# shaia/CFD

Measured on AMD Instinct MI355X. Metric: MLUPS + achieved HBM GB/s, 512^3 projection step, 1/2/4/8xMI355X, higher is better.
Workload: dtype f64

## Files before the change

### cfd_amd/csrc/hip/ccf.hpp

```cpp
#pragma once

#include "kernels.hpp"

namespace cfdhip {

#ifndef CFD_CCF_AHEAD
#define CFD_CCF_AHEAD 2
#endif
constexpr int CCF_AHEAD = CFD_CCF_AHEAD;
static_assert(CCF_AHEAD == 1 || CCF_AHEAD == 2, "k_ccf prefetch depth");
#ifndef CFD_CCF_CFIRST
#define CFD_CCF_CFIRST 0
#endif
constexpr bool CCF_CFIRST = CFD_CCF_CFIRST != 0;
#ifndef CFD_CCF_DIAG
#define CFD_CCF_DIAG 0
#endif
constexpr int CCF_DIAG = CFD_CCF_DIAG;
#ifndef CFD_CCF_NTST
#define CFD_CCF_NTST 1
#endif
constexpr bool CCF_NTST = CFD_CCF_NTST != 0;
#ifndef CFD_CCF_STAUX
#define CFD_CCF_STAUX (CFD_CCF_NTST ? 2 : 0)
#endif
constexpr int CCF_STAUX = CFD_CCF_STAUX;
#ifndef CFD_CCF_LDAUX
#define CFD_CCF_LDAUX 0
#endif
constexpr int CCF_LDAUX = CFD_CCF_LDAUX;
#ifndef CFD_CCF_NTFOLD
#define CFD_CCF_NTFOLD 0
#endif
constexpr bool CCF_NTFOLD = CFD_CCF_NTFOLD != 0;
constexpr int CCF_TC = 32;
constexpr int CCF_TR = 32;
constexpr int CCF_OX = 60;
constexpr int CCF_OY = 28;
constexpr int CCF_LP = CCF_TC + 2;
constexpr int CCF_LR = 2 * CCF_LP;
constexpr int CCF_LS = (CCF_TR + 2) * CCF_LR;
struct CcfLds {
    double pl[4][CCF_LS];
    double sh[32];
    int flag;
};

template <bool FIRST, bool FOLD, bool NOC = false>
static __global__ __launch_bounds__(1024, 4) void k_ccf(
    SGeo g, Lap Lp, const double* __restrict__ R0, double* __restrict__ R1,
    const double* __restrict__ Po, double* __restrict__ Pn, PPrev pv, double* __restrict__ x,
    CgState* st, double* partials, unsigned* counter, int it, int xmap, int dist, double* dsum,
    Mbox* mb, unsigned long long* clk) {
    static_assert(!(FIRST && FOLD), "k_ccf: no fold in the first iteration");
    __shared__ CcfLds L;
    if (CCF_DIAG == 0 && st->done) return;
    unsigned long long clk_t0 = 0, clk_r0 = 0;
    if (clk != nullptr && threadIdx.x < 64) {
        clk_t0 = __builtin_amdgcn_s_memtime();
        clk_r0 = __builtin_amdgcn_s_memrealtime();
        __builtin_amdgcn_s_waitcnt(0xC07F);
    }
    const double a = st->alpha[it % CG_XFOLD];
    const double ma = -a;
    const double beta = FIRST ? 0.0 : st->beta;
    double aq[CG_XFOLD - 1];
#pragma unroll
    for (int q = 0; q < CG_XFOLD - 1; ++q)
        aq[q] = FOLD ? st->alpha[(it + 1 + q) % CG_XFOLD] : 0.0;
    const int t = xmap ? xcd_tile(blockIdx.x, gridDim.x) : (int)blockIdx.x;
    const int tx = t % g.tiles_x;
    const int rest = t / g.tiles_x;
    const int ty = rest % g.tiles_y;
    const int tz = rest / g.tiles_y;
    const int lane = threadIdx.x & 63;
    const int w = __builtin_amdgcn_readfirstlane(threadIdx.x >> 6);
    const int c = lane & 31;
    const int r = w + 16 * (lane >> 5);
    const int i0 = tx * CCF_OX - 2 + 2 * c;
    const int j = ty * CCF_OY - 2 + r;
    int kb, ke;
    if (g.kmode == 1) {
        kb = (tz == 0) ? g.k0 : g.k1 - 1;
        ke = kb + 1;
    } else {
        const int kt0 = (g.kmode == 2) ? g.kt0 : g.k0;
        const int kt1 = (g.kmode == 2) ? g.kt1 : g.k1;
        if (tz < g.nz1) {
            kb = kt0 + tz * g.kc;
            ke = min(kb + g.kc, kt1);
        } else {
            kb = min(kt0 + g.nz1 * g.kc + (tz - g.nz1) * g.kc2, kt1);
            ke = min(kb + g.kc2, kt1);
        }
    }
    const bool jin = j >= 1 && j <= g.ny - 2;
    const bool in0 = jin && i0 >= 1 && i0 <= g.nx - 2;
    const bool in1 = jin && i0 + 1 >= 1 && i0 + 1 <= g.nx - 2;
    const bool own = c >= 1 && c <= CCF_TC - 2 && r >= 2 && r <= CCF_TR - 3;
    const bool wr = own && jin && i0 >= 0 && i0 < g.nx;
    const int ic = i0 < 0 ? 0 : (i0 < g.nx ? i0 : g.nx - 2 - ((g.nx - 2) & 1));
    const int col = max(min(j, g.ny - 1), 0) * (int)g.px + ic;
    auto plane = [&](int k) -> long long {
        return CCF_DIAG == 1 ? 0LL : (long long)min(max(k, 0), g.nz - 1) * g.ps;
    };
    double* const Lb = &L.pl[0][r * CCF_LR + c];
    constexpr int OWX = CCF_LR + 1, OWY = CCF_LR + 1 + CCF_LP;
    constexpr int LFo = CCF_LR + CCF_LP, RTo = CCF_LR + 2;
    constexpr int DNX = 1, DNY = 1 + CCF_LP, UPX = 2 * CCF_LR + 1, UPY = 2 * CCF_LR + 1 + CCF_LP;
    auto lrd = [&](int pl, int d) __attribute__((always_inline)) -> double {
        __builtin_amdgcn_sched_barrier(0x7ff);
        return Lb[pl * CCF_LS + d];
    };
    auto lput = [&](int pl, double2 v) __attribute__((always_inline)) {
        Lb[pl * CCF_LS + OWX] = v.x;
        Lb[pl * CCF_LS + OWY] = v.y;
    };
    for (int e = threadIdx.x; e < 4 * CCF_LS; e += 1024) {
        const int q = e % CCF_LS;
        const int row = q / CCF_LR, cc = q % CCF_LP;
        if (row == 0 || row == CCF_TR + 1 || cc == 0 || cc == CCF_LP - 1) L.pl[e / CCF_LS][q] = 0.0;
    }
    struct Nb {
        double lf, rt, dx, dy, ux, uy;
    };
    auto nbrs = [&](int pl) __attribute__((always_inline)) -> Nb {
        Nb n;
        n.lf = lrd(pl, LFo);
        n.rt = lrd(pl, RTo);
        n.dx = lrd(pl, DNX);
        n.dy = lrd(pl, DNY);
        n.ux = lrd(pl, UPX);
        n.uy = lrd(pl, UPY);
        return n;
    };
    auto stencil_n = [&](const Nb& n, double2 v, double2 zm, double2 zp, double2& out)
                         __attribute__((always_inline)) {
        out.x = -lap7(Lp, v.x, n.lf, v.y, n.dx, n.ux, zm.x, zp.x);
        out.y = -lap7(Lp, v.y, v.x, n.rt, n.dy, n.uy, zm.y, zp.y);
    };
    auto stencil = [&](int pl, double2 v, double2 zm, double2 zp, double2& out)
                       __attribute__((always_inline)) {
        if constexpr (CCF_DIAG == 2) {
            out.x = v.x + zm.x + zp.x;
            out.y = v.y + zm.y + zp.y;
        } else {
            stencil_n(nbrs(pl), v, zm, zp, out);
        }
    };
    const int q0 = kb - 4;
    const int nsteps = ke - kb + 4;
    double2 rr[4], po[4], pn[4], rn[4];
    double2 fx[2], f0[2], f1[2];
    const double2 zero = make_double2(0.0, 0.0);
#pragma unroll
    for (int s = 0; s < 4; ++s) pn[s] = rn[s] = po[s] = rr[s] = zero;
    fx[0] = fx[1] = f0[0] = f0[1] = f1[0] = f1[1] = zero;
    auto pro = [&](int k) __attribute__((always_inline)) {
        const int s = (k - q0) & 3;
        rr[s] = ld2ba<CCF_LDAUX>(R0 + plane(k), g.ps, col * 8);
        if (!FIRST) po[s] = ld2ba<CCF_LDAUX>(Po + plane(k), g.ps, col * 8);
        st2b<false>(Pn, g.ps, ST_NOSTORE, zero);
        st2b<false>(R1, g.ps, ST_NOSTORE, zero);
        if (FOLD) st2b<false>(x, g.ps, ST_NOSTORE, zero);
        __builtin_amdgcn_sched_barrier(0);
    };
    rr[2] = po[2] = zero;
    pro(q0 + 2);
    if (CCF_AHEAD == 2) pro(q0 + 3);
    double accg = 0.0, accd = 0.0;
    auto step = [&](auto Pc, int q) __attribute__((always_inline)) {
        constexpr int P = decltype(Pc)::value;
        constexpr int S0 = P & 3, S1 = (P + 1) & 3, S2 = (P + 2) & 3, S3 = (P + 3) & 3;
        constexpr int SM = (P + 3) & 3;
        constexpr int F1 = (P + 1) & 1, F2 = P & 1;
        constexpr int LPR = (P + 1) & 1, LPW = P & 1;
        constexpr int LRR = 2 + (P & 1), LRW = 2 + ((P + 1) & 1);
        __builtin_amdgcn_sched_barrier(0);
        {
            constexpr int SL = (CCF_AHEAD == 2) ? S0 : S3;
            const int ql = q + CCF_AHEAD + 2;
            const long long pbl = plane(ql);
            const int ol = (ql <= ke + 1) ? col * 8 : ST_NOSTORE;
            rr[SL] = ld2ba<CCF_LDAUX>(R0 + pbl, g.ps, ol);
            if (!FIRST) po[SL] = ld2ba<CCF_LDAUX>(Po + pbl, g.ps, ol);
        }
        if (FOLD) {
            const long long pb2 = plane(q + 2);
            const int o2 = (wr && q + 2 >= kb && q + 2 < ke) ? col * 8 : ST_NOSTORE;
            fx[F2] = ld2b<CCF_NTFOLD>(x + pb2, g.ps, o2);
            f0[F2] = ld2b<CCF_NTFOLD>(pv.q[0] + pb2, g.ps, o2);
            f1[F2] = ld2b<CCF_NTFOLD>(pv.q[1] + pb2, g.ps, o2);
        }
        __builtin_amdgcn_sched_barrier(0);
        __syncthreads();
        Nb nc{};
        if constexpr (!NOC && CCF_CFIRST) nc = nbrs(LRR);
        const double2 p2 = FIRST ? rr[S2] : fma2p(rr[S2], beta, po[S2]);
        pn[S2] = p2;
        double2 s;
        stencil(LPR, pn[S1], pn[S0], p2, s);
        const int qb = q + 1;
        const bool kbin = qb >= 1 && qb <= g.nz - 2;
        const double2 rv = rr[S1];
        const double2 r1 = make_double2((kbin && in0) ? rv.x + ma * s.x : 0.0,
                                        (kbin && in1) ? rv.y + ma * s.y : 0.0);
        rn[S1] = r1;
        if constexpr (!CCF_CFIRST) __builtin_amdgcn_sched_barrier(0);
        if constexpr (!NOC) {
            double2 wv;
            if constexpr (CCF_CFIRST) stencil_n(nc, rn[S0], rn[SM], r1, wv);
            else stencil(LRR, rn[S0], rn[SM], r1, wv);
            if (q >= kb && own) {
                const double2 rc = rn[S0];
                if (in0) {
                    accg += rc.x * rc.x;
                    accd += wv.x * rc.x;
                }
                if (in1) {
                    accg += rc.y * rc.y;
                    accd += wv.y * rc.y;
                }
            }
        }
        lput(LPW, p2);
        if constexpr (!NOC) lput(LRW, r1);
        {
            const bool qown = qb >= kb && qb < ke;
            const int bo = (qown && wr && CCF_DIAG != 1) ? col * 8 : ST_NOSTORE;
            const bool qhalo = NOC && ((qb == kb - 1 && kb == g.k0) || (qb == ke && ke == g.k1));
            const int bp = ((qown || qhalo) && wr && CCF_DIAG != 1) ? col * 8 : ST_NOSTORE;
            const long long pb = plane(qb);
            const double2 p1 = pn[S1];
            st2ba<CCF_STAUX>(Pn + pb, g.ps, bp, make_double2(in0 ? p1.x : 0.0, in1 ? p1.y : 0.0));
            st2ba<CCF_STAUX>(R1 + pb, g.ps, bo, r1);
            if (FOLD) {
                const double2 xo = fx[F1], qa = f0[F1], qq = f1[F1], qc = po[S1];
                double2 xw;
                xw.x = in0 ? (((xo.x + aq[0] * qa.x) + aq[1] * qq.x) + aq[2] * qc.x) + a * p1.x
                           : xo.x;
                xw.y = in1 ? (((xo.y + aq[0] * qa.y) + aq[1] * qq.y) + aq[2] * qc.y) + a * p1.y
                           : xo.y;
                st2ba<CCF_STAUX>(x + pb, g.ps, bo, xw);
            }
        }
        __builtin_amdgcn_sched_barrier(0);
    };
    int n = 0;
    for (; n + 3 < nsteps; n += 4) {
        step(IntC<0>{}, q0 + n);
        step(IntC<1>{}, q0 + n + 1);
        step(IntC<2>{}, q0 + n + 2);
        step(IntC<3>{}, q0 + n + 3);
    }
    if (n < nsteps) step(IntC<0>{}, q0 + n);
    if (n + 1 < nsteps) step(IntC<1>{}, q0 + n + 1);
    if (n + 2 < nsteps) step(IntC<2>{}, q0 + n + 2);
    if (clk != nullptr && threadIdx.x < 64) {
        const unsigned long long t1 = __builtin_amdgcn_s_memtime();
        const unsigned long long r1 = __builtin_amdgcn_s_memrealtime();
        __builtin_amdgcn_s_waitcnt(0xC07F);
        if (threadIdx.x == 0) {
            atomicAdd(&clk[0], t1 - clk_t0);
            atomicAdd(&clk[1], r1 - clk_r0);
            atomicAdd(&clk[2], 1ull);
        }
    }
    if constexpr (NOC) return;
    accg = wave_sum(accg);
    accd = wave_sum(accd);
    __syncthreads();
    if (lane == 0) {
        L.sh[w] = accg;
        L.sh[16 + w] = accd;
    }
    __syncthreads();
    double bg = 0.0, bd = 0.0;
    if (threadIdx.x == 0)
        for (int v = 0; v < 16; ++v) {
            bg += L.sh[v];
            bd += L.sh[16 + v];
        }
    double tg, td;
    double* shs = &L.pl[0][0];
    if (grid_sum2_last<1024>(bg, bd, partials, counter, shs, &L.flag, tg, td,
                             (unsigned)g.part_ofs, (unsigned)g.part_total) &&
        threadIdx.x == 0)
        cc_reduce_finish(st, tg, td, it, false, dist != 0, mb, dsum);
}

}
```

### cfd_amd/csrc/hip/ctx.hpp

```cpp
#pragma once

#include "kernels.hpp"
#include "slab_comm.hpp"

#include "cfd_hip/projection_hip.h"

#include <hip/hip_ext.h>
#include <hip/hip_runtime.h>

#include <algorithm>
#include <cmath>
#include <cstdio>
#include <cstdlib>
#include <cstring>
#include <initializer_list>
#include <vector>

using namespace cfdhip;

extern "C" void cfd_set_error(cfd_status_t status, const char* message) __attribute__((weak));

static inline void set_err(cfd_status_t s, const char* msg) {
    if (cfd_set_error) cfd_set_error(s, msg);
}
// ... 6 lines not shown
            snprintf(buf_, sizeof(buf_), "HIP error %s at %s:%d (%s)",             \
                     hipGetErrorString(e_), __FILE__, __LINE__, #call);            \
            set_err(CFD_ERROR, buf_);                                              \
            return CFD_ERROR;                                                      \
        }                                                                          \
    } while (0)

namespace {

struct TimedLaunch {
    hipEvent_t a, b;
    int kind;
    int iter;
};

}

struct hip_proj_ctx {
    int device = 0;
    hipStream_t stream = nullptr;
    size_t nx = 0, ny = 0, nz = 0;
    long long px = 0, ps = 0;
    Geo geo{};
    SGeo sgeo{};
    SGeo sg_edge{}, sg_int{};
    SGeo rgeo{};
    SGeo rg_in1{}, rg_edge{}, rg_in2{};
    int split_rb = 0;
    SGeo rg_main{}, rg_strip{};
    int rb_strip_tc = 0;
    int rb1_tc = 64;
    SGeo pgeo{};
    SGeo pgeo16{};
    int pc3 = 1;
    int split_b = 0;
    int sweep_ty = 8;
    int sweep_variant = 0;
    int sweep_variant_fold = 0;
    int grid_cap = 2048;
    hip_proj_config_t cfg{};
    SlabComm* comm = nullptr;
    int rank = 0, nranks = 1;
    size_t nzg = 0;
    size_t kofs = 0;
    double* dsum = nullptr;
    unsigned long long* clk = nullptr;
    hipStream_t hstream = nullptr;
    hipEvent_t ev_b = nullptr, ev_h = nullptr;
    unsigned long long* redg = nullptr;
    double *u = nullptr, *v = nullptr, *w = nullptr, *p = nullptr, *T = nullptr;
    double *us = nullptr, *vs = nullptr, *ws = nullptr, *pn = nullptr;
    double *r = nullptr, *pa = nullptr, *pb = nullptr;
    double *pc4 = nullptr, *pd4 = nullptr;
    double *rhs = nullptr, *xt = nullptr;
    int cg_scratch_dirty = 0;
    int poisson_bc = 0;
    double* bcfix = nullptr;
    int resident = 0;
    const double* res_ptr[5] = {nullptr, nullptr, nullptr, nullptr, nullptr};
    long long res_steps = 0;
    unsigned long long host_hash[5] = {0, 0, 0, 0, 0};
    unsigned long long host_hash1[5] = {0, 0, 0, 0, 0};
    int hash_ok = 0, hash_nf = 0;
    double* shell_dev = nullptr;
    double* shell_host = nullptr;
    size_t shell_cap = 0;
    double *cw = nullptr, *cs = nullptr;
    double* Tn = nullptr;
    double* rho = nullptr;
    double* rk_acc[4] = {nullptr, nullptr, nullptr, nullptr};
    double *dxa = nullptr, *dya = nullptr;
    double *src_u_row = nullptr, *src_v_col = nullptr;
    double* h_src = nullptr;
    hipEvent_t ev_src = nullptr;
    CgState* st = nullptr;
    RxState* rxst = nullptr;
    RxState* rxst2 = nullptr;
    void* rb2dec = nullptr;
    SGeo r2geo{};
    SGeo ccgeo{};
    SGeo cc_edge{}, cc_int{};
    SGeo cc_int_red{}, cc2_edge{};
    int ccf_tail = 0, ccf_kc2 = 0;
    std::vector<float> placement_ms;
    int placement_pick = -1;
    double* r2 = nullptr;
    double* partials = nullptr;
    unsigned* counter = nullptr;
    unsigned long long* red = nullptr;
    CgState* h_state = nullptr;
    unsigned long long* h_red = nullptr;
    hipEvent_t ev_poll[2] = {nullptr, nullptr};
    double rho0 = 1.0;
    double max_T = 0.0;
    int have_T = 0;
    int T_dirty = 0;
    poisson_solver_stats_t pstats{};
    size_t bytes = 0;
    std::vector<void*> allocs;
    size_t stagger_bytes = 0;
    struct {
        bool ccf_off = false;
        int cg_small = -1;
        int rb2_test = 0;
        int rb2_xmap = 0;
        bool rb2_log = false;
        int rb2 = 1;
        int ccf_xmap = 0;
        bool cgb_rev = true;
        bool rb1_pf = true;
        bool rb1_alt = true;
        bool rb1_fold = true;
        bool rk_pair = true;
        bool alloc_contig = false;
        bool ccf_edge_side = true;
    } env;
    int timing = 0;
    std::vector<hipEvent_t> ev_pool;
    size_t ev_used = 0;
    std::vector<TimedLaunch> pending;
    hipEvent_t ta = nullptr, tb = nullptr;
    double kt_ms[HIP_KT_COUNT] = {0};
    long long kt_n[HIP_KT_COUNT] = {0};
};

static cfd_status_t dalloc(hip_proj_ctx* c, double** ptr, size_t n) {
    const size_t off = (size_t)c->allocs.size() * c->stagger_bytes;
    void* base = nullptr;
    if (c->env.alloc_contig &&
        hipExtMallocWithFlags(&base, n * sizeof(double) + off, hipDeviceMallocContiguous) != hipSuccess) {
        (void)hipGetLastError();
        base = nullptr;
    }
    if (!base) HIP_TRY(hipMalloc(&base, n * sizeof(double) + off));
    c->allocs.push_back(base);
    *ptr = (double*)((char*)base + off);
    HIP_TRY(hipMemsetAsync(*ptr, 0, n * sizeof(double), c->stream));
    c->bytes += n * sizeof(double) + off;
    return CFD_SUCCESS;
}

static size_t field_elems(const hip_proj_ctx* c) { return (size_t)c->ps * c->nz; }

static double* field_ptr(hip_proj_ctx* c, int id) {
    switch (id) {
        case HIP_FIELD_U: return c->u;
        case HIP_FIELD_V: return c->v;
        case HIP_FIELD_W: return c->w;
        case HIP_FIELD_P: return c->p;
        case HIP_FIELD_T: return c->T;
        case HIP_FIELD_RHO: return c->rho;
        default: return nullptr;
    }
}

static hipEvent_t take_event(hip_proj_ctx* c) {
    if (c->ev_used == c->ev_pool.size()) {
        hipEvent_t e;
        if (hipEventCreate(&e) != hipSuccess) return nullptr;
        c->ev_pool.push_back(e);
    }
    return c->ev_pool[c->ev_used++];
}

static void flush_timing(hip_proj_ctx* c, int cg_limit = 0x7fffffff) {
    for (auto& t : c->pending) {
        if (t.iter >= cg_limit) continue;
        float ms = 0.f;
        if (hipEventElapsedTime(&ms, t.a, t.b) == hipSuccess) {
            c->kt_ms[t.kind] += ms;
            c->kt_n[t.kind] += 1;
        }
    }
    c->pending.clear();
    c->ev_used = 0;
}

template <typename F>
static void timed(hip_proj_ctx* c, int kind, F&& launch, int iter = -1) {
    if (!c->timing) {
        launch();
        return;
    }
    hipEvent_t a = take_event(c), b = take_event(c);
    if (!a || !b) {
        launch();
        return;
    }
    c->ta = a;
    c->tb = b;
    launch();
    c->ta = c->tb = nullptr;
    c->pending.push_back({a, b, kind, iter});
}

template <typename F>
static cfd_status_t timed_span(hip_proj_ctx* c, hipStream_t s, int kind, F&& fn, int iter = -1) {
    if (!c->timing) return fn();
// ... 143 lines not shown
```

### cfd_amd/csrc/hip/projection_hip.hip

```cpp
#include "ctx.hpp"

#include <array>
#include "rb2.hpp"
#include "ccf.hpp"

template <int TY, bool FIRST, bool DIST, int FL, bool FOLD>
static void launch_cgA_t(hip_proj_ctx* c, const Lap& L, const double* r, const double* po,
                         double* pn, int it, const PFold& fd) {
    hipExtLaunchKernelGGL((k_cgA<TY, FIRST, DIST, FL, FOLD>), dim3(sweep_grid(c)), dim3(64 * TY),
                          0, c->stream, c->ta, c->tb, 0, c->sgeo, L, r, po, pn, c->st, c->partials,
                          c->counter, it, c->dsum, mbox(c), fd);
}

struct BArgs {
    const double* p;
    double* r;
};

template <int TY, bool DIST, int FL>
static void launch_cgB_t(hip_proj_ctx* c, const SGeo& sg, const Lap& L, const BArgs& a, int it) {
    const unsigned nb = (unsigned)(sg.tiles_x * sg.tiles_y * sg.tiles_z);
    if (!DIST && c->env.cgb_rev && c->geo.sz && sg.kmode == 0) {
        hipExtLaunchKernelGGL((k_cgB<TY, DIST, FL, true>), dim3(nb), dim3(64 * TY), 0, c->stream,
                              c->ta, c->tb, 0, sg, L, a.p, a.r, c->st, c->partials, c->counter,
// ... 51 lines not shown
        case 4: return launch_cgB_f<TY, 4>(c, sg, L, a, it);
        case 7: return launch_cgB_f<TY, 7>(c, sg, L, a, it);
        case 15: return launch_cgB_f<TY, 15>(c, sg, L, a, it);
                 [[fallthrough]];
        case 23: if constexpr (TY == 16) return launch_cgB_f<TY, 23>(c, sg, L, a, it);
                 [[fallthrough]];
        case 31: if constexpr (TY == 16) return launch_cgB_f<TY, 31>(c, sg, L, a, it);
                 [[fallthrough]];
        default: return launch_cgB_f<TY, 0>(c, sg, L, a, it);
    }
}

static void launch_cgA(hip_proj_ctx* c, bool first, const Lap& L, const double* r,
                       const double* po, double* pn, int it, const PFold& fd) {
    if (c->sweep_ty == 4) return launch_cgA_f<4, 0>(c, first, L, r, po, pn, it, fd);
    if (c->sweep_ty == 16) return launch_cgA_v<16>(c, first, L, r, po, pn, it, fd);
    return launch_cgA_v<8>(c, first, L, r, po, pn, it, fd);
}

static void launch_cgB(hip_proj_ctx* c, const SGeo& sg, const Lap& L, const BArgs& a, int it) {
    if (c->sweep_ty == 4) return launch_cgB_f<4, 0>(c, sg, L, a, it);
    if (c->sweep_ty == 16) return launch_cgB_v<16>(c, sg, L, a, it);
    return launch_cgB_v<8>(c, sg, L, a, it);
}

template <bool FIRST, bool FOLD>
static void launch_cc1_t(hip_proj_ctx* c, double* pn, const double* po, const PPrev& pv, double* x,
                         int it) {
    const unsigned n = (unsigned)(c->px / 2) * (unsigned)(c->ny - 2) *
                       (unsigned)(c->sgeo.k1 - c->sgeo.k0);
    const unsigned nb = std::max(1u, std::min((n + 255) / 256, (unsigned)c->grid_cap * 4));
    hipExtLaunchKernelGGL((k_cc1<FIRST, FOLD>), dim3(nb), dim3(256), 0, c->stream, c->ta, c->tb, 0,
                          c->sgeo, c->r, c->cw, c->cs, po, pn, pv, x, c->st, it);
}

static void launch_cc1(hip_proj_ctx* c, double* pn, const double* po, const PPrev& pv, double* x,
                       int it) {
    const bool fold = (it % CG_XFOLD) == CG_XFOLD - 1;
    if (it == 0) launch_cc1_t<true, false>(c, pn, po, pv, x, it);
    else if (fold) launch_cc1_t<false, true>(c, pn, po, pv, x, it);
    else launch_cc1_t<false, false>(c, pn, po, pv, x, it);
}

template <int TY, bool DIST, bool INIT, bool WST>
static void launch_cc2_t(hip_proj_ctx* c, const SGeo& g, const Lap& L, int it, const double* r) {
    const unsigned nb = (unsigned)(g.tiles_x * g.tiles_y * g.tiles_z);
    hipExtLaunchKernelGGL((k_cc2<TY, DIST, INIT, WST>), dim3(nb), dim3(64 * TY), 0,
                          c->stream, c->ta, c->tb, 0, g, L, r, c->cw, c->st, c->partials,
                          c->counter, it, c->dsum, mbox(c));
}

template <int TY, bool WST>
static void launch_cc2_w(hip_proj_ctx* c, const SGeo& g, const Lap& L, int it, bool init,
                         const double* r) {
    if (dist(c)) init ? launch_cc2_t<TY, true, true, WST>(c, g, L, it, r)
                      : launch_cc2_t<TY, true, false, WST>(c, g, L, it, r);
    else init ? launch_cc2_t<TY, false, true, WST>(c, g, L, it, r)
              : launch_cc2_t<TY, false, false, WST>(c, g, L, it, r);
}

template <int TY>
static void launch_cc2_ty(hip_proj_ctx* c, const SGeo& g, const Lap& L, int it, bool init,
                          const double* r, bool wst) {
    wst ? launch_cc2_w<TY, true>(c, g, L, it, init, r)
        : launch_cc2_w<TY, false>(c, g, L, it, init, r);
}

static void launch_cc2(hip_proj_ctx* c, const Lap& L, int it, bool init, const double* r,
                       bool wst, const SGeo* gp = nullptr) {
    const SGeo& g = gp ? *gp : c->sgeo;
    if (c->sweep_ty == 16) return launch_cc2_ty<16>(c, g, L, it, init, r, wst);
    if (c->sweep_ty == 4) return launch_cc2_ty<4>(c, g, L, it, init, r, wst);
    return launch_cc2_ty<8>(c, g, L, it, init, r, wst);
}

static const double* ccf_r0(const hip_proj_ctx* c, int it) { return (it & 1) ? c->r2 : c->r; }
static double* ccf_r1(hip_proj_ctx* c, int it) { return (it & 1) ? c->r : c->r2; }

template <bool FIRST, bool FOLD, bool NOC>
static void launch_ccf_t(hip_proj_ctx* c, const SGeo& g, const Lap& L, double* pn,
                         const double* po, const PPrev& pv, double* x, int it, int xmap,
                         hipStream_t s) {
    unsigned long long* clk = (c->timing && c->clk && (it & 5) == 5) ? c->clk : nullptr;
    hipExtLaunchKernelGGL((k_ccf<FIRST, FOLD, NOC>), dim3(g.tiles_x * g.tiles_y * g.tiles_z),
                          dim3(1024), 0, s, c->ta, c->tb, 0, g, L, ccf_r0(c, it),
                          ccf_r1(c, it), po, pn, pv, x, c->st, c->partials, c->counter, it, xmap,
                          dist(c) ? 1 : 0, c->dsum, mbox(c), clk);
}

template <bool NOC>
static void launch_ccf_n(hip_proj_ctx* c, const SGeo& g, const Lap& L, double* pn,
                         const double* po, const PPrev& pv, double* x, int it, int xmap,
                         hipStream_t s) {
    const bool fold = (it % CG_XFOLD) == CG_XFOLD - 1;
    if (it == 0) launch_ccf_t<true, false, NOC>(c, g, L, pn, po, pv, x, it, xmap, s);
    else if (fold) launch_ccf_t<false, true, NOC>(c, g, L, pn, po, pv, x, it, xmap, s);
    else launch_ccf_t<false, false, NOC>(c, g, L, pn, po, pv, x, it, xmap, s);
}

static void launch_ccf(hip_proj_ctx* c, const SGeo& g, const Lap& L, double* pn,
                       const double* po, const PPrev& pv, double* x, int it, bool noc,
                       hipStream_t s = nullptr) {
    const int xmap = c->env.ccf_xmap;
    if (!s) s = c->stream;
    if (noc) launch_ccf_n<true>(c, g, L, pn, po, pv, x, it, xmap, s);
    else launch_ccf_n<false>(c, g, L, pn, po, pv, x, it, xmap, s);
}

enum RhsSource { RHS_FROM_VELOCITY, RHS_FROM_ARRAY };

static cfd_status_t cg_solve(hip_proj_ctx* c, double dx, double dy, double dz,
                             const DivCoef& dc, RhsSource src, double rel_tol, double abs_tol,
                             int max_iter, int check_interval, bool final_bc) {
    const Lap L = make_lap(dx, dy, dz);
    const int G = tile_grid(c);
    const DirVals dv{};
    const bool D = dist(c);
    double* x = c->pn;
    if (c->cg_scratch_dirty) {
        for (double* f : {c->r, c->pa, c->pb, c->pc4, c->pd4, c->r2})
            if (f) HIP_TRY(hipMemsetAsync(f, 0, field_elems(c) * sizeof(double), c->stream));
        c->cg_scratch_dirty = 0;
    }
    ST_TRY(halo(c, {x}));
    const bool neumann = (c->poisson_bc == HIP_POISSON_BC_NEUMANN);
    if (neumann) launch_bc(c, x, 0, dv);
    timed(c, HIP_KT_CG_SETUP, [&] {
        const double* rhs_in = (src == RHS_FROM_VELOCITY) ? nullptr : c->rhs;
        if (src == RHS_FROM_VELOCITY) {
            if (D)
                hipExtLaunchKernelGGL((k_cg_setup<true, false, true, true>), dim3(G), dim3(NT), 0,
                                   c->stream, c->ta, c->tb, 0, c->geo, L, dc, c->us, c->vs, c->ws, nullptr, x,
                                   c->r, c->st, c->partials, c->counter, rel_tol, abs_tol,
                                   max_iter, check_interval, c->dsum, mbox(c));
            else
                hipExtLaunchKernelGGL((k_cg_setup<true, false, true, false>), dim3(G), dim3(NT), 0,
                                   c->stream, c->ta, c->tb, 0, c->geo, L, dc, c->us, c->vs, c->ws, nullptr, x,
                                   c->r, c->st, c->partials, c->counter, rel_tol, abs_tol,
                                   max_iter, check_interval, c->dsum, (Mbox*)nullptr);
        } else {
            if (D)
                hipExtLaunchKernelGGL((k_cg_setup<false, false, true, true>), dim3(G), dim3(NT), 0,
                                   c->stream, c->ta, c->tb, 0, c->geo, L, dc, nullptr, nullptr, nullptr,
                                   (double*)rhs_in, x, c->r, c->st, c->partials, c->counter,
                                   rel_tol, abs_tol, max_iter, check_interval, c->dsum, mbox(c));
            else
                hipExtLaunchKernelGGL((k_cg_setup<false, false, true, false>), dim3(G), dim3(NT), 0,
                                   c->stream, c->ta, c->tb, 0, c->geo, L, dc, nullptr, nullptr, nullptr,
                                   (double*)rhs_in, x, c->r, c->st, c->partials, c->counter,
                                   rel_tol, abs_tol, max_iter, check_interval, c->dsum, (Mbox*)nullptr);
        }
    });
    if (D && !mbox(c)) {
        ST_TRY(reduce_dot(c));
        hipExtLaunchKernelGGL(k_finish_setup, dim3(1), dim3(64), 0, c->stream, c->ta, c->tb, 0,
                              c->st, c->dsum + 1, rel_tol, abs_tol, max_iter, check_interval);
    }
    if (D) ST_TRY(halo(c, {c->r}));
    double* P[CG_XFOLD] = {c->pa, c->pb, c->pc4, c->pd4};
    auto iterate = [&](int it) -> cfd_status_t {
        double* pnew = P[it % CG_XFOLD];
        double* pold = P[(it + CG_XFOLD - 1) % CG_XFOLD];
        const bool fold = it > 0 && (it % CG_XFOLD) == 0;
        const PFold fd{P[(it + 1) % CG_XFOLD], P[(it + 2) % CG_XFOLD], fold ? x : nullptr};
        const BArgs ba{pnew, c->r};
        const int kb = HIP_KT_CG_SWEEP_B;
        const int ka = fold ? HIP_KT_CG_SWEEP_BX : HIP_KT_CG_SWEEP_A;
        timed(c, ka, [&] { launch_cgA(c, it == 0, L, c->r, pold, pnew, it, fd); }, it);
        if (D && !mbox(c)) {
            ST_TRY(timed_span(c, c->stream, HIP_KT_ALLREDUCE, [&] {
// ... 760 lines not shown
}

int hip_projection_available(void) {
    int n = 0;
    if (hipGetDeviceCount(&n) != hipSuccess) return 0;
    return n > 0 ? 1 : 0;
}

static void free_ctx(hip_proj_ctx* c) {
    if (!c) return;
    if (c->stream) hipStreamSynchronize(c->stream);
    for (void* b : c->allocs) hipFree(b);
    if (c->st) hipFree(c->st);
    if (c->rxst) hipFree(c->rxst);
    if (c->rxst2) hipFree(c->rxst2);
    if (c->rb2dec) hipFree(c->rb2dec);
    if (c->partials) hipFree(c->partials);
    if (c->counter) hipFree(c->counter);
    if (c->red) hipFree(c->red);
    if (c->redg) hipFree(c->redg);
    if (c->dsum) hipFree(c->dsum);
    if (c->clk) hipFree(c->clk);
    if (c->h_state) hipHostFree(c->h_state);
    if (c->h_red) hipHostFree(c->h_red);
    if (c->h_src) hipHostFree(c->h_src);
    if (c->ev_src) hipEventDestroy(c->ev_src);
    if (c->shell_host) hipHostFree(c->shell_host);
    if (c->shell_dev) hipFree(c->shell_dev);
    for (int i = 0; i < 2; i++)
        if (c->ev_poll[i]) hipEventDestroy(c->ev_poll[i]);
    for (auto e : c->ev_pool) hipEventDestroy(e);
    if (c->ev_b) hipEventDestroy(c->ev_b);
    if (c->ev_h) hipEventDestroy(c->ev_h);
    if (c->hstream) {
        hipStreamSynchronize(c->hstream);
        hipStreamDestroy(c->hstream);
    }
    if (c->stream) hipStreamDestroy(c->stream);
    delete c;
}

static void ccf_layout(SGeo& g, int P, int kc, int kc2, int tail_layers) {
    kc = std::max(1, std::min(kc, P));
    g.kc = kc;
    g.kc2 = kc;
    g.nz1 = g.tiles_z = (P + kc - 1) / kc;
    if (tail_layers <= 0 || kc2 <= 0 || kc2 >= kc) return;
    const int tail = std::min(P, tail_layers * kc2);
    const int bulk = P - tail;
    if (bulk <= 0) return;
    g.kc2 = kc2;
    g.nz1 = (bulk + kc - 1) / kc;
    const int rest = std::max(0, P - g.nz1 * kc);
    g.tiles_z = g.nz1 + (rest + kc2 - 1) / kc2;
}

static cfd_status_t init_ctx(hip_proj_ctx* c, size_t nx, size_t ny, size_t nz) {
    HIP_TRY(hipSetDevice(c->device));
    HIP_TRY(hipStreamCreateWithFlags(&c->stream, hipStreamNonBlocking));
    hipDeviceProp_t prop;
    HIP_TRY(hipGetDeviceProperties(&prop, c->device));
    c->grid_cap = std::max(64, prop.multiProcessorCount * 8);
    c->stagger_bytes = (c->cfg.cg_variant == 1) ? 4096 : 0;
    if (const char* e = getenv("CFD_HIP_FIELD_STAGGER")) c->stagger_bytes = (size_t)atol(e) / 256 * 256;
    {
        auto ienv = [](const char* name, int dflt) {
            const char* e = getenv(name);
            return e ? atoi(e) : dflt;
        };
        c->env.ccf_off = ienv("CFD_HIP_CCF", 1) == 0;
        c->env.cg_small = ienv("CFD_HIP_CG_SMALL", -1);
        c->env.rb2_test = ienv("CFD_HIP_RB2_TEST", 0);
        c->env.rb2_xmap = ienv("CFD_HIP_RB2_XMAP", 0);
        c->env.rb2_log = getenv("CFD_HIP_RB2_LOG") != nullptr;
        c->env.rb2 = ienv("CFD_HIP_RB2", 1);
        c->env.ccf_xmap = ienv("CFD_HIP_CCF_XMAP", 0);
        c->env.cgb_rev = ienv("CFD_HIP_CGB_REV", 1) != 0;
        c->env.rb1_pf = ienv("CFD_HIP_RB1_PF", 1) != 0;
        c->env.rb1_alt = ienv("CFD_HIP_RB1_ALT", 1) != 0;
        c->env.rb1_fold = ienv("CFD_HIP_RB1_FOLD", 1) != 0;
        c->env.rk_pair = ienv("CFD_HIP_RK_PAIR", 1) != 0;
        c->env.alloc_contig = getenv("CFD_HIP_ALLOC") && strcmp(getenv("CFD_HIP_ALLOC"), "contig") == 0;
        c->env.ccf_edge_side = ienv("CFD_HIP_CCF_EDGE_SIDE", 1) != 0;
    }
    c->nx = nx;
    c->ny = ny;
    c->nz = nz;
    c->px = (long long)((nx + 7) / 8 * 8);
    if (const char* e = getenv("CFD_HIP_ROW_PAD")) c->px += (long long)(std::max(0, atoi(e)) / 8 * 8);
    c->ps = c->px * (long long)ny;
    Geo& g = c->geo;
    g.nx = (int)nx;
    g.ny = (int)ny;
    g.nz = (int)nz;
    g.px = c->px;
    g.ps = c->ps;
    g.sz = (nz > 1) ? c->ps : 0;
    g.k0 = (nz > 1) ? 1 : 0;
    g.k1 = (nz > 1) ? (int)nz - 1 : 1;
    g.lo_face = (c->rank == 0) ? 1 : 0;
    g.hi_face = (c->rank == c->nranks - 1) ? 1 : 0;
    g.kofs = (int)c->kofs;
    const int nint_k = g.k1 - g.k0;
    int kc = 0;
    if (kc <= 0) {
        long long xy_tiles = (long long)((nx + TX - 1) / TX) * (long long)((ny + TY - 1) / TY);
        long long want = 4LL * c->grid_cap;
        kc = (int)std::max<long long>(8, (xy_tiles * nint_k + want - 1) / want);
        kc = std::min(kc, std::max(1, nint_k));
    }
    g.kc = std::max(1, kc);
    g.tiles_x = (int)((nx + TX - 1) / TX);
    g.tiles_y = (int)((ny + TY - 1) / TY);
    g.tiles_z = (nint_k + g.kc - 1) / g.kc;

    c->sweep_ty = (c->cfg.sweep_rows == 4 || c->cfg.sweep_rows == 16) ? c->cfg.sweep_rows : 8;
    {
        const int v = c->cfg.sweep_variant & 63;
        if (v == 15 && c->sweep_ty >= 8) c->sweep_variant = v;
        else if ((v == 23 || v == 31) && c->sweep_ty == 16) c->sweep_variant = v;
        else c->sweep_variant = (v & SW_PREFETCH) ? ((v & 3) == 3 ? 7 : 4) : (v & 3);
    }
    {
        const int vf = c->cfg.sweep_variant_fold;
        c->sweep_variant_fold = (c->sweep_ty == 16 && (vf == 3 || vf == 11 || vf == 15)) ? vf : 0;
    }
    SGeo& sg = c->sgeo;
    sg.nx = g.nx;
    sg.ny = g.ny;
    sg.nz = g.nz;
    sg.px = g.px;
    sg.ps = g.ps;
    sg.sz = g.sz;
    sg.k0 = g.k0;
    sg.k1 = g.k1;
    sg.kofs = g.kofs;
    sg.tiles_x = (int)((nx + 127) / 128);
    sg.tiles_y = (int)((ny + c->sweep_ty - 1) / c->sweep_ty);
    if (c->cfg.kchunk > 0) {
        sg.kc = c->cfg.kchunk;
    } else {
        sg.kc = 256;
        const long long want = c->grid_cap / 8;
        while (sg.kc > 4 &&
               (long long)sg.tiles_x * sg.tiles_y * ((nint_k + sg.kc - 1) / sg.kc) < want)
            sg.kc /= 2;
    }
    sg.kc = std::max(1, std::min(sg.kc, nint_k));
    sg.tiles_z = (nint_k + sg.kc - 1) / sg.kc;
    int n_partials = std::max(c->grid_cap, sg.tiles_x * sg.tiles_y * sg.tiles_z);
    {
        SGeo& rg = c->rgeo;
        rg = sg;
        int tc = 64;
        if (const char* e = getenv("CFD_HIP_RB1_TC")) {
            const int v = atoi(e);
            if (v == 64 || v == 32 || v == 16) tc = v;
        }
        c->rb1_tc = tc;
        const int ox = 2 * tc - 4, oy = 1024 / tc - 4;
        rg.tiles_x = (int)((nx - 1 + ox - 1) / ox);
        rg.tiles_y = (int)((ny - 1 + oy - 1) / oy);
        rg.kc = 64;
        if (const char* e = getenv("CFD_HIP_RB1_KC")) rg.kc = std::max(1, atoi(e));
        while (rg.kc > 16 &&
               (long long)rg.tiles_x * rg.tiles_y * ((nint_k + rg.kc - 1) / rg.kc) < 512)
            rg.kc /= 2;
        while (rg.kc > 4 &&
               (long long)rg.tiles_x * rg.tiles_y * ((nint_k + rg.kc - 1) / rg.kc) < 128)
            rg.kc /= 2;
        rg.kc = std::max(1, std::min(rg.kc, nint_k));
        rg.tiles_z = (nint_k + rg.kc - 1) / rg.kc;
        n_partials = std::max(n_partials, rg.tiles_x * rg.tiles_y * rg.tiles_z);
        SGeo& r2 = c->r2geo;
        r2 = rg;
        r2.tiles_x = r2.tiles_y = r2.tiles_z = 0;
        if (c->nranks == 1 && nz > 1 && nx >= 8 && ny >= 8) {
            r2.xofs = 0;
            r2.tiles_x = (int)((nx - 1 + RB2_OX - 1) / RB2_OX);
            r2.tiles_y = (int)((ny - 1 + RB2_OY - 1) / RB2_OY);
            r2.kc = 128;
            if (nint_k >= 384 &&
                3LL * r2.tiles_x * r2.tiles_y >= 8LL * std::max(1, c->grid_cap / 8))
                r2.kc = (nint_k + 2) / 3;
            if (const char* e = getenv("CFD_HIP_RB2_KC")) r2.kc = std::max(1, atoi(e));
            while (r2.kc > 4 &&
                   (long long)r2.tiles_x * r2.tiles_y * ((nint_k + r2.kc - 1) / r2.kc) < 512)
                r2.kc /= 2;
            r2.kc = std::max(1, std::min(r2.kc, nint_k));
            r2.tiles_z = (nint_k + r2.kc - 1) / r2.kc;
            n_partials = std::max(n_partials, 2 * r2.tiles_x * r2.tiles_y * r2.tiles_z);
        }
        SGeo& cg = c->ccgeo;
        cg = rg;
        cg.tiles_x = cg.tiles_y = cg.tiles_z = 0;
        if (nz >= 3 && nx >= 4 && ny >= 4) {
            cg.xofs = 0;
            cg.tiles_x = (int)((nx - 1 + CCF_OX - 1) / CCF_OX);
            cg.tiles_y = (int)((ny - 1 + CCF_OY - 1) / CCF_OY);
            cg.kc = (c->nranks == 1) ? 24 : (nint_k <= 100 ? 11 : 16);
            const char* ekc = getenv("CFD_HIP_CCF_KC");
            if (ekc) cg.kc = std::max(1, atoi(ekc));
            const bool kc_fixed = getenv("CFD_HIP_CCF_KC_FIXED") != nullptr;
            while (!kc_fixed && cg.kc > 4 &&
                   (long long)cg.tiles_x * cg.tiles_y * ((nint_k + cg.kc - 1) / cg.kc) < 512)
                cg.kc /= 2;
            const int tail_l = getenv("CFD_HIP_CCF_TAIL") ? atoi(getenv("CFD_HIP_CCF_TAIL")) : 0;
            const int kc2 = getenv("CFD_HIP_CCF_KC2") ? atoi(getenv("CFD_HIP_CCF_KC2")) : cg.kc / 2;
            c->ccf_tail = tail_l;
            c->ccf_kc2 = kc2;
            ccf_layout(cg, nint_k, cg.kc, kc2, tail_l);
            n_partials = std::max(n_partials, cg.tiles_x * cg.tiles_y * cg.tiles_z);
            c->cc_edge = c->cc_int = cg;
            c->cc_edge.tiles_x = c->cc_int.tiles_x = 0;
            if (c->nranks > 1 && nint_k >= 3) {
                SGeo& e = c->cc_edge;
                SGeo& m = c->cc_int;
                e = m = cg;
                e.kmode = 1;
                e.kc = 1;
                e.tiles_z = 2;
                m.kmode = 2;
                m.kt0 = cg.k0 + 1;
                m.kt1 = cg.k1 - 1;
                ccf_layout(m, m.kt1 - m.kt0, cg.kc, c->ccf_kc2, c->ccf_tail);
                const char* ef = getenv("CFD_HIP_CCF_SLAB_FUSED");
                if (!(ef && atoi(ef) == 0)) {
                    SGeo& ir = c->cc_int_red;
                    SGeo& ee = c->cc2_edge;
                    ir = m;
                    ee = sg;
                    ee.kmode = 1;
                    ee.kc = 1;
                    ee.tiles_z = 2;
                    const int ni = ir.tiles_x * ir.tiles_y * ir.tiles_z;
                    const int ne = ee.tiles_x * ee.tiles_y * ee.tiles_z;
                    ir.part_ofs = 0;
                    ee.part_ofs = ni;
                    ir.part_total = ee.part_total = ni + ne;
                    n_partials = std::max(n_partials, ni + ne);
                }
            }
        }
        const char* estrip = getenv("CFD_HIP_RB1_STRIP");
        c->rb_strip_tc = 0;
        if (tc == 64 && c->nranks == 1 && !(estrip && atoi(estrip) == 0)) {
            const int T = (int)(nx / 124), R = (int)nx - 124 * T;
            const int stc = (R >= 2 && R <= 28) ? 16 : 0;
            if (stc) {
                c->rb_strip_tc = stc;
                SGeo& m = c->rg_main;
                SGeo& q = c->rg_strip;
                m = rg;
                m.tiles_x = T;
                q = rg;
                q.xofs = 124 * T;
                q.tiles_x = 1;
                const int oy = 1024 / stc - 4;
                q.tiles_y = (int)((ny - 1 + oy - 1) / oy);
                q.kc = std::max(1, std::min(rg.kc, nint_k));
                q.tiles_z = (nint_k + q.kc - 1) / q.kc;
                m.part_ofs = q.part_ofs = 0;
                m.part_total = q.part_total = 0;
                n_partials = std::max(n_partials, m.tiles_x * m.tiles_y * m.tiles_z +
                                                      q.tiles_x * q.tiles_y * q.tiles_z);
            }
        }
        const char* es = getenv("CFD_HIP_RB_SPLIT");
        c->split_rb = (c->nranks > 1 && nint_k >= 4 && !(es && atoi(es) == 0)) ? 1 : 0;
        if (c->split_rb) {
            const int a0 = g.k0 + 1, a1 = g.k1 - 1;
            const int mid = a0 + (a1 - a0) / 2;
            auto range = [&](SGeo& q, int lo, int hi) {
                q = rg;
                q.kmode = 2;
                q.kt0 = lo;
                q.kt1 = hi;
                q.kc = std::max(1, std::min(rg.kc, hi - lo));
                q.tiles_z = (hi - lo + q.kc - 1) / q.kc;
            };
            range(c->rg_in1, a0, mid);
            range(c->rg_in2, mid, a1);
// ... 1105 lines not shown
```

Before: 135.9.

## Compute CG curvature dot product via edge-difference form in fused CCF kernel

Adds an EDGE variant of the fused CG kernel that computes r·Ar as a sum of squared edge differences plus wall terms, instead of applying the full 7-point stencil to the new residual. This needs only one-sided neighbours, so the y halo shrinks by one row (tile output height grows from 28 to 29), the z prologue shortens, and the rn ring buffer shrinks. It is enabled by default on single rank with interior k-mode. It trades fewer tiles and less stencil work for a reformulated reduction whose rounding differs, and it depends on the wall-term handling being correct.

After: 138.3, median of 6. 1.8% higher.

```diff
diff --git a/cfd_amd/csrc/hip/ccf.hpp b/cfd_amd/csrc/hip/ccf.hpp
--- a/cfd_amd/csrc/hip/ccf.hpp
+++ b/cfd_amd/csrc/hip/ccf.hpp
@@ -37,6 +37,7 @@
 constexpr int CCF_TR = 32;
 constexpr int CCF_OX = 60;
 constexpr int CCF_OY = 28;
+constexpr int CCF_OY_EDGE = 29;
 constexpr int CCF_LP = CCF_TC + 2;
 constexpr int CCF_LR = 2 * CCF_LP;
 constexpr int CCF_LS = (CCF_TR + 2) * CCF_LR;
@@ -46,13 +47,17 @@
     int flag;
 };
 
-template <bool FIRST, bool FOLD, bool NOC = false>
-static __global__ __launch_bounds__(1024, 4) void k_ccf(
-    SGeo g, Lap Lp, const double* __restrict__ R0, double* __restrict__ R1,
+template <bool FIRST, bool FOLD, bool NOC, bool EDGE>
+static __device__ __forceinline__ void ccf_body(
+    const SGeo& g, const Lap& Lp, const double* __restrict__ R0, double* __restrict__ R1,
     const double* __restrict__ Po, double* __restrict__ Pn, PPrev pv, double* __restrict__ x,
     CgState* st, double* partials, unsigned* counter, int it, int xmap, int dist, double* dsum,
     Mbox* mb, unsigned long long* clk) {
     static_assert(!(FIRST && FOLD), "k_ccf: no fold in the first iteration");
+    static_assert(!(NOC && EDGE), "k_ccf: the edge sum is stage c's");
+    constexpr int OY = EDGE ? CCF_OY_EDGE : CCF_OY;
+    constexpr int RLO = EDGE ? 1 : 2;
+    constexpr int ZPRO = EDGE ? 3 : 4;
     __shared__ CcfLds L;
     if (CCF_DIAG == 0 && st->done) return;
     unsigned long long clk_t0 = 0, clk_r0 = 0;
@@ -78,7 +83,7 @@
     const int c = lane & 31;
     const int r = w + 16 * (lane >> 5);
     const int i0 = tx * CCF_OX - 2 + 2 * c;
-    const int j = ty * CCF_OY - 2 + r;
+    const int j = ty * OY - RLO + r;
     int kb, ke;
     if (g.kmode == 1) {
         kb = (tz == 0) ? g.k0 : g.k1 - 1;
@@ -97,7 +102,7 @@
     const bool jin = j >= 1 && j <= g.ny - 2;
     const bool in0 = jin && i0 >= 1 && i0 <= g.nx - 2;
     const bool in1 = jin && i0 + 1 >= 1 && i0 + 1 <= g.nx - 2;
-    const bool own = c >= 1 && c <= CCF_TC - 2 && r >= 2 && r <= CCF_TR - 3;
+    const bool own = c >= 1 && c <= CCF_TC - 2 && r >= RLO && r <= CCF_TR - 3;
     const bool wr = own && jin && i0 >= 0 && i0 < g.nx;
     const int ic = i0 < 0 ? 0 : (i0 < g.nx ? i0 : g.nx - 2 - ((g.nx - 2) & 1));
     const int col = max(min(j, g.ny - 1), 0) * (int)g.px + ic;
@@ -148,13 +153,18 @@
             stencil_n(nbrs(pl), v, zm, zp, out);
         }
     };
-    const int q0 = kb - 4;
-    const int nsteps = ke - kb + 4;
-    double2 rr[4], po[4], pn[4], rn[4];
+    const int q0 = kb - ZPRO;
+    const int nsteps = ke - kb + ZPRO;
+    const double wal0 = (EDGE && j == 1) ? Lp.dy2_inv : 0.0;
+    const double wal1 = (EDGE && i0 == 0) ? wal0 + Lp.dx2_inv : wal0;
+    constexpr int RNM = EDGE ? 1 : 3;
+    double2 rr[4], po[4], pn[4], rn[RNM + 1];
     double2 fx[2], f0[2], f1[2];
     const double2 zero = make_double2(0.0, 0.0);
 #pragma unroll
-    for (int s = 0; s < 4; ++s) pn[s] = rn[s] = po[s] = rr[s] = zero;
+    for (int s = 0; s < 4; ++s) pn[s] = po[s] = rr[s] = zero;
+#pragma unroll
+    for (int s = 0; s <= RNM; ++s) rn[s] = zero;
     fx[0] = fx[1] = f0[0] = f0[1] = f1[0] = f1[1] = zero;
     auto pro = [&](int k) __attribute__((always_inline)) {
         const int s = (k - q0) & 3;
@@ -173,6 +183,7 @@
         constexpr int P = decltype(Pc)::value;
         constexpr int S0 = P & 3, S1 = (P + 1) & 3, S2 = (P + 2) & 3, S3 = (P + 3) & 3;
         constexpr int SM = (P + 3) & 3;
+        constexpr int RS0 = P & RNM, RS1 = (P + 1) & RNM;
         constexpr int F1 = (P + 1) & 1, F2 = P & 1;
         constexpr int LPR = (P + 1) & 1, LPW = P & 1;
         constexpr int LRR = 2 + (P & 1), LRW = 2 + ((P + 1) & 1);
@@ -195,7 +206,12 @@
         __builtin_amdgcn_sched_barrier(0);
         __syncthreads();
         Nb nc{};
-        if constexpr (!NOC && CCF_CFIRST) nc = nbrs(LRR);
+        if constexpr (!NOC && !EDGE && CCF_CFIRST) nc = nbrs(LRR);
+        if constexpr (EDGE && CCF_CFIRST) {
+            nc.rt = lrd(LRR, RTo);
+            nc.ux = lrd(LRR, UPX);
+            nc.uy = lrd(LRR, UPY);
+        }
         const double2 p2 = FIRST ? rr[S2] : fma2p(rr[S2], beta, po[S2]);
         pn[S2] = p2;
         double2 s;
@@ -205,14 +221,38 @@
         const double2 rv = rr[S1];
         const double2 r1 = make_double2((kbin && in0) ? rv.x + ma * s.x : 0.0,
                                         (kbin && in1) ? rv.y + ma * s.y : 0.0);
-        rn[S1] = r1;
+        rn[RS1] = r1;
         if constexpr (!CCF_CFIRST) __builtin_amdgcn_sched_barrier(0);
-        if constexpr (!NOC) {
+        if constexpr (EDGE) {
+            if constexpr (!CCF_CFIRST && CCF_DIAG != 2) {
+                nc.rt = lrd(LRR, RTo);
+                nc.ux = lrd(LRR, UPX);
+                nc.uy = lrd(LRR, UPY);
+            }
+            if (q >= kb && own) {
+                const double2 rc = rn[RS0];
+                const double walz = (q == 1) ? Lp.inv_dz2 : 0.0;
+                if (in0) {
+                    const double g2 = rc.x * rc.x;
+                    const double ex = rc.x - rc.y, ey = rc.x - nc.ux, ez = rc.x - r1.x;
+                    accg += g2;
+                    accd += ((Lp.dx2_inv * (ex * ex) + Lp.dy2_inv * (ey * ey)) +
+                             Lp.inv_dz2 * (ez * ez)) + (wal0 + walz) * g2;
+                }
+                if (in1) {
+                    const double g2 = rc.y * rc.y;
+                    const double ex = rc.y - nc.rt, ey = rc.y - nc.uy, ez = rc.y - r1.y;
+                    accg += g2;
+                    accd += ((Lp.dx2_inv * (ex * ex) + Lp.dy2_inv * (ey * ey)) +
+                             Lp.inv_dz2 * (ez * ez)) + (wal1 + walz) * g2;
+                }
+            }
+        } else if constexpr (!NOC) {
             double2 wv;
-            if constexpr (CCF_CFIRST) stencil_n(nc, rn[S0], rn[SM], r1, wv);
-            else stencil(LRR, rn[S0], rn[SM], r1, wv);
+            if constexpr (CCF_CFIRST) stencil_n(nc, rn[RS0], rn[SM], r1, wv);
+            else stencil(LRR, rn[RS0], rn[SM], r1, wv);
             if (q >= kb && own) {
-                const double2 rc = rn[S0];
+                const double2 rc = rn[RS0];
                 if (in0) {
                     accg += rc.x * rc.x;
                     accd += wv.x * rc.x;
@@ -289,4 +329,24 @@
         cc_reduce_finish(st, tg, td, it, false, dist != 0, mb, dsum);
 }
 
+template <bool FIRST, bool FOLD, bool NOC = false>
+static __global__ __launch_bounds__(1024, 4) void k_ccf(
+    SGeo g, Lap Lp, const double* __restrict__ R0, double* __restrict__ R1,
+    const double* __restrict__ Po, double* __restrict__ Pn, PPrev pv, double* __restrict__ x,
+    CgState* st, double* partials, unsigned* counter, int it, int xmap, int dist, double* dsum,
+    Mbox* mb, unsigned long long* clk) {
+    ccf_body<FIRST, FOLD, NOC, !NOC>(g, Lp, R0, R1, Po, Pn, pv, x, st, partials, counter, it, xmap,
+                                     dist, dsum, mb, clk);
 }
+
+template <bool FIRST, bool FOLD>
+static __global__ __launch_bounds__(1024, 4) void k_ccf_cell(
+    SGeo g, Lap Lp, const double* __restrict__ R0, double* __restrict__ R1,
+    const double* __restrict__ Po, double* __restrict__ Pn, PPrev pv, double* __restrict__ x,
+    CgState* st, double* partials, unsigned* counter, int it, int xmap, int dist, double* dsum,
+    Mbox* mb, unsigned long long* clk) {
+    ccf_body<FIRST, FOLD, false, false>(g, Lp, R0, R1, Po, Pn, pv, x, st, partials, counter, it,
+                                        xmap, dist, dsum, mb, clk);
+}
+
+}
diff --git a/cfd_amd/csrc/hip/ctx.hpp b/cfd_amd/csrc/hip/ctx.hpp
--- a/cfd_amd/csrc/hip/ctx.hpp
+++ b/cfd_amd/csrc/hip/ctx.hpp
@@ -112,6 +112,7 @@
     SGeo cc_edge{}, cc_int{};
     SGeo cc_int_red{}, cc2_edge{};
     int ccf_tail = 0, ccf_kc2 = 0;
+    bool ccf_edge_dot = false;
     std::vector<float> placement_ms;
     int placement_pick = -1;
     double* r2 = nullptr;
@@ -144,6 +145,7 @@
         bool rk_pair = true;
         bool alloc_contig = false;
         bool ccf_edge_side = true;
+        bool ccf_edge_dot = true;
     } env;
     int timing = 0;
     std::vector<hipEvent_t> ev_pool;
diff --git a/cfd_amd/csrc/hip/projection_hip.hip b/cfd_amd/csrc/hip/projection_hip.hip
--- a/cfd_amd/csrc/hip/projection_hip.hip
+++ b/cfd_amd/csrc/hip/projection_hip.hip
@@ -157,10 +157,19 @@
                          const double* po, const PPrev& pv, double* x, int it, int xmap,
                          hipStream_t s) {
     unsigned long long* clk = (c->timing && c->clk && (it & 5) == 5) ? c->clk : nullptr;
-    hipExtLaunchKernelGGL((k_ccf<FIRST, FOLD, NOC>), dim3(g.tiles_x * g.tiles_y * g.tiles_z),
-                          dim3(1024), 0, s, c->ta, c->tb, 0, g, L, ccf_r0(c, it),
-                          ccf_r1(c, it), po, pn, pv, x, c->st, c->partials, c->counter, it, xmap,
-                          dist(c) ? 1 : 0, c->dsum, mbox(c), clk);
+    const bool cell = !NOC && !(c->ccf_edge_dot && g.kmode == 0);
+    const dim3 grid(g.tiles_x * g.tiles_y * g.tiles_z);
+    if (cell) {
+        if constexpr (!NOC)
+            hipExtLaunchKernelGGL((k_ccf_cell<FIRST, FOLD>), grid, dim3(1024), 0, s, c->ta, c->tb,
+                                  0, g, L, ccf_r0(c, it), ccf_r1(c, it), po, pn, pv, x, c->st,
+                                  c->partials, c->counter, it, xmap, dist(c) ? 1 : 0, c->dsum,
+                                  mbox(c), clk);
+        return;
+    }
+    hipExtLaunchKernelGGL((k_ccf<FIRST, FOLD, NOC>), grid, dim3(1024), 0, s, c->ta, c->tb, 0, g,
+                          L, ccf_r0(c, it), ccf_r1(c, it), po, pn, pv, x, c->st, c->partials,
+                          c->counter, it, xmap, dist(c) ? 1 : 0, c->dsum, mbox(c), clk);
 }
 
 template <bool NOC>
@@ -1087,6 +1096,7 @@
         c->env.rk_pair = ienv("CFD_HIP_RK_PAIR", 1) != 0;
         c->env.alloc_contig = getenv("CFD_HIP_ALLOC") && strcmp(getenv("CFD_HIP_ALLOC"), "contig") == 0;
         c->env.ccf_edge_side = ienv("CFD_HIP_CCF_EDGE_SIDE", 1) != 0;
+        c->env.ccf_edge_dot = ienv("CFD_HIP_CCF_EDGE_DOT", 1) != 0;
     }
     c->nx = nx;
     c->ny = ny;
@@ -1196,13 +1206,15 @@
             r2.tiles_z = (nint_k + r2.kc - 1) / r2.kc;
             n_partials = std::max(n_partials, 2 * r2.tiles_x * r2.tiles_y * r2.tiles_z);
         }
+        c->ccf_edge_dot = c->nranks == 1 && c->env.ccf_edge_dot;
+        const int ccf_oy = c->ccf_edge_dot ? CCF_OY_EDGE : CCF_OY;
         SGeo& cg = c->ccgeo;
         cg = rg;
         cg.tiles_x = cg.tiles_y = cg.tiles_z = 0;
         if (nz >= 3 && nx >= 4 && ny >= 4) {
             cg.xofs = 0;
             cg.tiles_x = (int)((nx - 1 + CCF_OX - 1) / CCF_OX);
-            cg.tiles_y = (int)((ny - 1 + CCF_OY - 1) / CCF_OY);
+            cg.tiles_y = (int)((ny - 1 + ccf_oy - 1) / ccf_oy);
             cg.kc = (c->nranks == 1) ? 24 : (nint_k <= 100 ? 11 : 16);
             const char* ekc = getenv("CFD_HIP_CCF_KC");
             if (ekc) cg.kc = std::max(1, atoi(ekc));
```
